# lbcb-sci/herro

Measured on NVIDIA H100. Metric: corrected_bases_per_sec, higher is better.
Workload: dtype u8 pileup/consensus + f32 forward

## Files before the change

### herro_b200/csrc/gemm_tc.cu

```cuda
#include <cstdio>
#include <cuda.h>
#include <cuda_bf16.h>

#include "common.cuh"
#include "forward.h"

namespace hb {

namespace {

constexpr int BM = 128, BN = 128, BK = 64, STAGES = 3;
constexpr int STAGE_BYTES = (2 * BM + 2 * BN) * 128;
constexpr int C_THREADS = 256, G_THREADS = 288, G_PROD_WARP = 8;

__device__ __forceinline__ uint32_t smem_u32(const void* p) { return (uint32_t)__cvta_generic_to_shared(p); }

__device__ __forceinline__ void mbar_init(uint64_t* bar, uint32_t count) {
    asm volatile("mbarrier.init.shared::cta.b64 [%0], %1;" ::"r"(smem_u32(bar)), "r"(count));
}
__device__ __forceinline__ void mbar_arrive(uint64_t* bar) {
    asm volatile("{\n\t.reg .b64 st;\n\tmbarrier.arrive.shared::cta.b64 st, [%0];\n\t}" ::"r"(smem_u32(bar)) : "memory");
}
__device__ __forceinline__ void mbar_wait(uint64_t* bar, uint32_t parity) {
    asm volatile(
        "{\n\t"
        ".reg .pred p;\n\t"
        "WAIT_LOOP:\n\t"
        "mbarrier.try_wait.parity.shared::cta.b64 p, [%0], %1;\n\t"
        "@p bra WAIT_DONE;\n\t"
        "bra WAIT_LOOP;\n\t"
        "WAIT_DONE:\n\t"
        "}" ::"r"(smem_u32(bar)), "r"(parity)
        : "memory");
}
__device__ __forceinline__ void mbar_arrive_expect_tx(uint64_t* bar, uint32_t bytes) {
    asm volatile("mbarrier.arrive.expect_tx.shared::cta.b64 _, [%0], %1;" ::"r"(smem_u32(bar)), "r"(bytes) : "memory");
}
__device__ __forceinline__ void tma_load_2d(uint32_t dst, const CUtensorMap* tm, uint64_t* bar, int c_inner, int c_row) {
    asm volatile("cp.async.bulk.tensor.2d.shared::cluster.global.mbarrier::complete_tx::bytes [%0], [%1, {%3, %4}], [%2];" ::"r"(dst),
                 "l"((uint64_t)tm), "r"(smem_u32(bar)), "r"(c_inner), "r"(c_row)
                 : "memory");
}
__device__ __forceinline__ void bar_sync(int id, int n) { asm volatile("bar.sync %0, %1;" ::"r"(id), "r"(n) : "memory"); }
__device__ __forceinline__ void fence_async_smem() { asm volatile("fence.proxy.async.shared::cta;" ::: "memory"); }

__device__ __forceinline__ uint64_t make_desc(uint32_t saddr) {
    uint64_t d = 0;
    d |= (uint64_t)((saddr & 0x3ffffu) >> 4);
    d |= (uint64_t)1 << 16;
    d |= (uint64_t)(1024u >> 4) << 32;
    d |= (uint64_t)1 << 62;
    return d;
}

__device__ __forceinline__ void wg_fence() { asm volatile("wgmma.fence.sync.aligned;" ::: "memory"); }
__device__ __forceinline__ void wg_commit() { asm volatile("wgmma.commit_group.sync.aligned;" ::: "memory"); }
template <int N>
__device__ __forceinline__ void wg_wait() { asm volatile("wgmma.wait_group.sync.aligned %0;" ::"n"(N) : "memory"); }
template <int R>
__device__ __forceinline__ void acc_fence(float (&a)[R]) {
#pragma unroll
    for (int i = 0; i < R; i++) asm volatile("" : "+f"(a[i])::"memory");
}

__device__ __forceinline__ void wgmma_n128(float (&d)[64], uint64_t adesc, uint64_t bdesc, uint32_t accumulate) {
    asm volatile(
        "{\n\t.reg .pred p;\n\tsetp.ne.b32 p, %66, 0;\n\t"
        "wgmma.mma_async.sync.aligned.m64n128k16.f32.bf16.bf16 "
        "{%0, %1, %2, %3, %4, %5, %6, %7, %8, %9, %10, %11, %12, %13, %14, %15, %16, %17, %18, %19, %20, %21, %22, %23, %24, %25, %26, %27, %28, %29, %30, %31, %32, %33, %34, %35, %36, %37, %38, %39, %40, %41, %42, %43, %44, %45, %46, %47, %48, %49, %50, %51, %52, %53, %54, %55, %56, %57, %58, %59, %60, %61, %62, %63}, "
        "%64, %65, p, 1, 1, 0, 0;\n\t}"
        : "+f"(d[0]), "+f"(d[1]), "+f"(d[2]), "+f"(d[3]), "+f"(d[4]), "+f"(d[5]), "+f"(d[6]), "+f"(d[7]), "+f"(d[8]), "+f"(d[9]), "+f"(d[10]), "+f"(d[11]), "+f"(d[12]), "+f"(d[13]), "+f"(d[14]), "+f"(d[15]), "+f"(d[16]), "+f"(d[17]), "+f"(d[18]), "+f"(d[19]), "+f"(d[20]), "+f"(d[21]), "+f"(d[22]), "+f"(d[23]), "+f"(d[24]), "+f"(d[25]), "+f"(d[26]), "+f"(d[27]), "+f"(d[28]), "+f"(d[29]), "+f"(d[30]), "+f"(d[31]), "+f"(d[32]), "+f"(d[33]), "+f"(d[34]), "+f"(d[35]), "+f"(d[36]), "+f"(d[37]), "+f"(d[38]), "+f"(d[39]), "+f"(d[40]), "+f"(d[41]), "+f"(d[42]), "+f"(d[43]), "+f"(d[44]), "+f"(d[45]), "+f"(d[46]), "+f"(d[47]), "+f"(d[48]), "+f"(d[49]), "+f"(d[50]), "+f"(d[51]), "+f"(d[52]), "+f"(d[53]), "+f"(d[54]), "+f"(d[55]), "+f"(d[56]), "+f"(d[57]), "+f"(d[58]), "+f"(d[59]), "+f"(d[60]), "+f"(d[61]), "+f"(d[62]), "+f"(d[63])
        : "l"(adesc), "l"(bdesc), "r"(accumulate)
        : "memory");
}
__device__ __forceinline__ void wgmma_n128_ra(float (&d)[64], uint32_t a0, uint32_t a1, uint32_t a2, uint32_t a3, uint64_t bdesc) {
    asm volatile(
        "wgmma.mma_async.sync.aligned.m64n128k16.f32.bf16.bf16 "
        "{%0, %1, %2, %3, %4, %5, %6, %7, %8, %9, %10, %11, %12, %13, %14, %15, %16, %17, %18, %19, %20, %21, %22, %23, %24, %25, %26, %27, %28, %29, %30, %31, %32, %33, %34, %35, %36, %37, %38, %39, %40, %41, %42, %43, %44, %45, %46, %47, %48, %49, %50, %51, %52, %53, %54, %55, %56, %57, %58, %59, %60, %61, %62, %63}, "
        "{%64, %65, %66, %67}, %68, 1, 1, 1, 0;"
        : "+f"(d[0]), "+f"(d[1]), "+f"(d[2]), "+f"(d[3]), "+f"(d[4]), "+f"(d[5]), "+f"(d[6]), "+f"(d[7]), "+f"(d[8]), "+f"(d[9]), "+f"(d[10]), "+f"(d[11]), "+f"(d[12]), "+f"(d[13]), "+f"(d[14]), "+f"(d[15]), "+f"(d[16]), "+f"(d[17]), "+f"(d[18]), "+f"(d[19]), "+f"(d[20]), "+f"(d[21]), "+f"(d[22]), "+f"(d[23]), "+f"(d[24]), "+f"(d[25]), "+f"(d[26]), "+f"(d[27]), "+f"(d[28]), "+f"(d[29]), "+f"(d[30]), "+f"(d[31]), "+f"(d[32]), "+f"(d[33]), "+f"(d[34]), "+f"(d[35]), "+f"(d[36]), "+f"(d[37]), "+f"(d[38]), "+f"(d[39]), "+f"(d[40]), "+f"(d[41]), "+f"(d[42]), "+f"(d[43]), "+f"(d[44]), "+f"(d[45]), "+f"(d[46]), "+f"(d[47]), "+f"(d[48]), "+f"(d[49]), "+f"(d[50]), "+f"(d[51]), "+f"(d[52]), "+f"(d[53]), "+f"(d[54]), "+f"(d[55]), "+f"(d[56]), "+f"(d[57]), "+f"(d[58]), "+f"(d[59]), "+f"(d[60]), "+f"(d[61]), "+f"(d[62]), "+f"(d[63])
        : "r"(a0), "r"(a1), "r"(a2), "r"(a3), "l"(bdesc)
        : "memory");
}
__device__ __forceinline__ void wgmma_n96(float (&d)[48], uint64_t adesc, uint64_t bdesc, uint32_t accumulate) {
    asm volatile(
        "{\n\t.reg .pred p;\n\tsetp.ne.b32 p, %50, 0;\n\t"
        "wgmma.mma_async.sync.aligned.m64n96k16.f32.bf16.bf16 "
        "{%0, %1, %2, %3, %4, %5, %6, %7, %8, %9, %10, %11, %12, %13, %14, %15, %16, %17, %18, %19, %20, %21, %22, %23, %24, %25, %26, %27, %28, %29, %30, %31, %32, %33, %34, %35, %36, %37, %38, %39, %40, %41, %42, %43, %44, %45, %46, %47}, "
        "%48, %49, p, 1, 1, 0, 0;\n\t}"
        : "+f"(d[0]), "+f"(d[1]), "+f"(d[2]), "+f"(d[3]), "+f"(d[4]), "+f"(d[5]), "+f"(d[6]), "+f"(d[7]), "+f"(d[8]), "+f"(d[9]), "+f"(d[10]), "+f"(d[11]), "+f"(d[12]), "+f"(d[13]), "+f"(d[14]), "+f"(d[15]), "+f"(d[16]), "+f"(d[17]), "+f"(d[18]), "+f"(d[19]), "+f"(d[20]), "+f"(d[21]), "+f"(d[22]), "+f"(d[23]), "+f"(d[24]), "+f"(d[25]), "+f"(d[26]), "+f"(d[27]), "+f"(d[28]), "+f"(d[29]), "+f"(d[30]), "+f"(d[31]), "+f"(d[32]), "+f"(d[33]), "+f"(d[34]), "+f"(d[35]), "+f"(d[36]), "+f"(d[37]), "+f"(d[38]), "+f"(d[39]), "+f"(d[40]), "+f"(d[41]), "+f"(d[42]), "+f"(d[43]), "+f"(d[44]), "+f"(d[45]), "+f"(d[46]), "+f"(d[47])
        : "l"(adesc), "l"(bdesc), "r"(accumulate)
        : "memory");
}

__device__ __forceinline__ void mma_kblock(float (&acc)[64], uint32_t a_hi, uint32_t a_lo, uint32_t b_hi, uint32_t b_lo, bool zero) {
    const uint64_t dAh = make_desc(a_hi), dAl = make_desc(a_lo), dBh = make_desc(b_hi), dBl = make_desc(b_lo);
// ... 319 lines not shown
        if (FUSE_O) {
            issue(accO, 0, true);
            issue(accO, 1, true);
            ffn_retire<1>(empty_bar, it_stage);
            acc_fence(accO);
#pragma unroll
            for (int j = 0; j < 16; j++) {
                const int c = 8 * j + fc;
                const float2 x0 = xr[2 * j], x1 = xr[2 * j + 1];
                accO[4 * j] = accO[4 * j] + s_bo[c] + x0.x; accO[4 * j + 1] = accO[4 * j + 1] + s_bo[c + 1] + x0.y;
                accO[4 * j + 2] = accO[4 * j + 2] + s_bo[c] + x1.x; accO[4 * j + 3] = accO[4 * j + 3] + s_bo[c + 1] + x1.y;
            }
            float ln[4];
            frag_ln_stats(accO, ln[0], ln[1], ln[2], ln[3]);
            bar_sync(1 + wg, 128);
            frag_store_tile(accO, sA1, fr, fc, s_ln2g, s_ln2b, ln);
#pragma unroll
            for (int j = 0; j < 16; j++) {
                const int c = 8 * j + fc;
                accO[4 * j] += s_b2[c]; accO[4 * j + 1] += s_b2[c + 1]; accO[4 * j + 2] += s_b2[c]; accO[4 * j + 3] += s_b2[c + 1];
            }
            fence_async_smem();
            bar_sync(1 + wg, 128);
        }
        issue(accF, 0, true);
        issue(accF, 1, true);
        ffn_retire<1>(empty_bar, it_stage);
        acc_fence(accF);
        e1(0);
        for (int c = 0; c < 3; c++) {
            issue_f2();
            issue(accF, 0, true);
            issue(accF, 1, true);
            ffn_retire<3>(empty_bar, it_stage);
            acc_fence(accF);
            reg_fence(ahi);
            reg_fence(alo);
            if (c == 2) mbar_arrive(&a1_empty);
            e1(c + 1);
        }
        issue_f2();
        ffn_retire<1>(empty_bar, it_stage);
        acc_fence(accO);
        reg_fence(ahi);
        reg_fence(alo);
        if (g.store_x) frag_store_f32(accO, g.X, BN, row0, 0, fc);
        frag_layernorm(accO, s_lng, s_lnb, fc);
        frag_store_split(accO, g.out_hi, g.out_lo, BN, row0, 0, fc);
    }
}

constexpr int QA_HROWS = 96;
constexpr int QA_RING_BYTES = 2 * QA_HROWS * 128;
constexpr int QA_STAGES = 3;
constexpr int QA_POS_BYTES = 6 * 2048;

__device__ __forceinline__ void ldsm_x4(uint32_t addr, uint32_t (&r)[4]) {
    asm volatile("ldmatrix.sync.aligned.m8n8.x4.shared.b16 {%0, %1, %2, %3}, [%4];" : "=r"(r[0]), "=r"(r[1]), "=r"(r[2]), "=r"(r[3]) : "r"(addr));
}
__device__ __forceinline__ void ldsm_x4_trans(uint32_t addr, uint32_t (&r)[4]) {
    asm volatile("ldmatrix.sync.aligned.m8n8.x4.trans.shared.b16 {%0, %1, %2, %3}, [%4];" : "=r"(r[0]), "=r"(r[1]), "=r"(r[2]), "=r"(r[3]) : "r"(addr));
}
__device__ __forceinline__ void mma16816(float (&c)[4], const uint32_t (&a)[4], uint32_t b0, uint32_t b1) {
    asm volatile("mma.sync.aligned.m16n8k16.row.col.f32.bf16.bf16.f32 {%0, %1, %2, %3}, {%4, %5, %6, %7}, {%8, %9}, {%0, %1, %2, %3};"
                 : "+f"(c[0]), "+f"(c[1]), "+f"(c[2]), "+f"(c[3])
                 : "r"(a[0]), "r"(a[1]), "r"(a[2]), "r"(a[3]), "r"(b0), "r"(b1));
}
__device__ __forceinline__ uint32_t qa_off(int row, int chunk) { return (uint32_t)(row * 64 + ((chunk ^ ((row >> 1) & 3)) << 4)); }

__global__ void __launch_bounds__(G_THREADS, 1) k_qkv_attn_ws(QkvAttnArgs g, const __grid_constant__ CUtensorMap tmHhi,
                                                             const __grid_constant__ CUtensorMap tmHlo, const __grid_constant__ CUtensorMap tmWhi,
                                                             const __grid_constant__ CUtensorMap tmWlo) {
    extern __shared__ uint8_t smem_dyn[];
    uint8_t* smem = smem_dyn + ((1024u - (smem_u32(smem_dyn) & 1023u)) & 1023u);
    uint8_t* sA = smem;
    uint8_t* ring = sA + FFN_A_BYTES;
    uint8_t* sP = ring + QA_STAGES * QA_RING_BYTES;
    __shared__ uint64_t full_bar[QA_STAGES], empty_bar[QA_STAGES], a_full, a_empty;
    __shared__ __align__(16) float s_bias[4 * QA_HROWS];

    const int tid = threadIdx.x, warp = tid >> 5, lane = tid & 31;
    if (tid == 0) {
        for (int s = 0; s < QA_STAGES; s++) { mbar_init(&full_bar[s], 1); mbar_init(&empty_bar[s], C_THREADS); }
        mbar_init(&a_full, 1); mbar_init(&a_empty, C_THREADS);
        asm volatile("fence.mbarrier_init.release.cluster;" ::: "memory");
    }
    for (int i = tid; i < 4 * QA_HROWS; i += G_THREADS) s_bias[i] = g.bias[i];
    __syncthreads();

    if (warp == G_PROD_WARP) {
        if (lane == 0) {
            uint32_t it_stage = 0, n_done = 0;
            for (uint32_t tile = blockIdx.x; tile < g.m_tiles; tile += gridDim.x, n_done++) {
                const int m0 = (int)(tile * BM);
                mbar_wait(&a_empty, (n_done & 1) ^ 1);
                mbar_arrive_expect_tx(&a_full, FFN_A_BYTES);
                for (int kb = 0; kb < 2; kb++) {
                    tma_load_2d(smem_u32(sA) + kb * (2 * BM * 128), &tmHhi, &a_full, kb * BK, m0);
                    tma_load_2d(smem_u32(sA) + kb * (2 * BM * 128) + BM * 128, &tmHlo, &a_full, kb * BK, m0);
                }
                for (int h = 0; h < 4; h++)
                    for (int kb = 0; kb < 2; kb++, it_stage++) {
                        const uint32_t s = it_stage % QA_STAGES, ph = (it_stage / QA_STAGES) & 1;
                        mbar_wait(&empty_bar[s], ph ^ 1);
                        const uint32_t sb = smem_u32(ring + (size_t)s * QA_RING_BYTES);
                        mbar_arrive_expect_tx(&full_bar[s], QA_RING_BYTES);
                        tma_load_2d(sb, &tmWhi, &full_bar[s], kb * BK, h * QA_HROWS);
                        tma_load_2d(sb + QA_HROWS * 128, &tmWlo, &full_bar[s], kb * BK, h * QA_HROWS);
                    }
            }
        }
        return;
    }
    const int wg = warp >> 2;
    const int pos = wg * 2 + ((warp & 3) >> 1);
    const int mt = warp & 1;
    const int gq = lane >> 2, tq = lane & 3;
    uint8_t* pb = sP + (size_t)pos * QA_POS_BYTES;
    uint8_t *aQh = pb, *aQl = pb + 2048, *aKh = pb + 4096, *aKl = pb + 6144, *aVh = pb + 8192, *aVl = pb + 10240;
    const uint32_t uQh = smem_u32(aQh), uQl = smem_u32(aQl), uKh = smem_u32(aKh), uKl = smem_u32(aKl), uVh = smem_u32(aVh),
                   uVl = smem_u32(aVl);
    const float scale_l2 = rsqrtf(32.f) * 1.4426950408889634f;
    const uint32_t ab = smem_u32(sA) + wg * 64 * 128;
    uint32_t it_stage = 0, n_done = 0;
    for (uint32_t tile = blockIdx.x; tile < g.m_tiles; tile += gridDim.x, n_done++) {
        mbar_wait(&a_full, n_done & 1);
        for (int h = 0; h < 4; h++) {
            float acc[48];
            for (int kb = 0; kb < 2; kb++, it_stage++) {
                const uint32_t s = it_stage % QA_STAGES, ph = (it_stage / QA_STAGES) & 1;
                mbar_wait(&full_bar[s], ph);
                const uint32_t sb = smem_u32(ring + (size_t)s * QA_RING_BYTES);
                const uint32_t a = ab + kb * (2 * BM * 128);
                const uint64_t dAh = make_desc(a), dAl = make_desc(a + BM * 128), dBh = make_desc(sb), dBl = make_desc(sb + QA_HROWS * 128);
                wg_fence();
#pragma unroll
                for (int k = 0; k < BK / 16; k++) {
                    const uint64_t adv = (uint64_t)(k * 2);
                    wgmma_n96(acc, dAh + adv, dBh + adv, (kb | k) ? 1u : 0u);
                    wgmma_n96(acc, dAl + adv, dBh + adv, 1u);
                    wgmma_n96(acc, dAh + adv, dBl + adv, 1u);
                }
                wg_commit();
            }
            wg_wait<0>();
            acc_fence(acc);
            mbar_arrive(&empty_bar[(it_stage - 2) % QA_STAGES]);
            mbar_arrive(&empty_bar[(it_stage - 1) % QA_STAGES]);
            if (h == 3) mbar_arrive(&a_empty);
            bar_sync(3 + pos, 64);
            const float* bb = s_bias + h * QA_HROWS;
#pragma unroll
            for (int j = 0; j < 12; j++) {
                const int c = 8 * j + 2 * tq;
                const float sc = j < 4 ? scale_l2 : 1.f;
                uint8_t* hi_arr = j < 4 ? aQh : (j < 8 ? aKh : aVh);
                const int cc = c & 31;
#pragma unroll
                for (int hf = 0; hf < 2; hf++) {
                    const int row = mt * 16 + hf * 8 + gq;
                    uint32_t hw, lw;
                    split2((acc[4 * j + 2 * hf] + bb[c]) * sc, (acc[4 * j + 2 * hf + 1] + bb[c + 1]) * sc, hw, lw);
                    const uint32_t off = qa_off(row, cc >> 3) + (cc & 7) * 2;
                    *(uint32_t*)(hi_arr + off) = hw;
                    *(uint32_t*)(hi_arr + 2048 + off) = lw;
                }
            }
            bar_sync(3 + pos, 64);
            float sacc[4][4];
#pragma unroll
            for (int nt = 0; nt < 4; nt++)
#pragma unroll
                for (int e = 0; e < 4; e++) sacc[nt][e] = 0.f;
            {
                uint32_t qh[2][4], ql[2][4];
#pragma unroll
                for (int ks = 0; ks < 2; ks++) {
                    const uint32_t off = qa_off(mt * 16 + (lane & 7) + ((lane >> 3) & 1) * 8, ks * 2 + (lane >> 4));
                    ldsm_x4(uQh + off, qh[ks]);
                    ldsm_x4(uQl + off, ql[ks]);
                }
#pragma unroll
                for (int ntp = 0; ntp < 2; ntp++)
#pragma unroll
                    for (int ks = 0; ks < 2; ks++) {
                        uint32_t kh[4], kl[4];
                        const uint32_t off = qa_off(ntp * 16 + (lane & 7) + (lane >> 4) * 8, ks * 2 + ((lane >> 3) & 1));
                        ldsm_x4(uKh + off, kh);
                        ldsm_x4(uKl + off, kl);
#pragma unroll
                        for (int j = 0; j < 2; j++) {
                            mma16816(sacc[ntp * 2 + j], qh[ks], kh[2 * j], kh[2 * j + 1]);
                            mma16816(sacc[ntp * 2 + j], ql[ks], kh[2 * j], kh[2 * j + 1]);
                            mma16816(sacc[ntp * 2 + j], qh[ks], kl[2 * j], kl[2 * j + 1]);
                        }
                    }
            }
            float inv[2];
#pragma unroll
            for (int hf = 0; hf < 2; hf++) {
                if (tq == 3) sacc[3][2 * hf + 1] = -INFINITY;
                float m = -INFINITY;
#pragma unroll
                for (int nt = 0; nt < 4; nt++) m = fmaxf(m, fmaxf(sacc[nt][2 * hf], sacc[nt][2 * hf + 1]));
                m = fmaxf(m, __shfl_xor_sync(HB_FULL, m, 1));
                m = fmaxf(m, __shfl_xor_sync(HB_FULL, m, 2));
                float l = 0.f;
#pragma unroll
                for (int nt = 0; nt < 4; nt++) {
                    const float p0 = exp2f(sacc[nt][2 * hf] - m), p1 = exp2f(sacc[nt][2 * hf + 1] - m);
                    sacc[nt][2 * hf] = p0; sacc[nt][2 * hf + 1] = p1;
                    l += p0 + p1;
                }
                l += __shfl_xor_sync(HB_FULL, l, 1);
                l += __shfl_xor_sync(HB_FULL, l, 2);
                const int row = mt * 16 + hf * 8 + gq;
                inv[hf] = (row < R_COLS) ? 1.f / l : 0.f;
            }
            float oacc[4][4];
#pragma unroll
            for (int dt = 0; dt < 4; dt++)
#pragma unroll
                for (int e = 0; e < 4; e++) oacc[dt][e] = 0.f;
#pragma unroll
            for (int ks = 0; ks < 2; ks++) {
                uint32_t ph[4], pl[4];
                split2(sacc[2 * ks][0], sacc[2 * ks][1], ph[0], pl[0]);
                split2(sacc[2 * ks][2], sacc[2 * ks][3], ph[1], pl[1]);
                split2(sacc[2 * ks + 1][0], sacc[2 * ks + 1][1], ph[2], pl[2]);
                split2(sacc[2 * ks + 1][2], sacc[2 * ks + 1][3], ph[3], pl[3]);
#pragma unroll
                for (int dp = 0; dp < 2; dp++) {
                    uint32_t vh[4], vl[4];
                    const uint32_t off = qa_off(ks * 16 + (lane & 7) + ((lane >> 3) & 1) * 8, dp * 2 + (lane >> 4));
                    ldsm_x4_trans(uVh + off, vh);
                    ldsm_x4_trans(uVl + off, vl);
#pragma unroll
                    for (int j = 0; j < 2; j++) {
                        mma16816(oacc[dp * 2 + j], ph, vh[2 * j], vh[2 * j + 1]);
                        mma16816(oacc[dp * 2 + j], pl, vh[2 * j], vh[2 * j + 1]);
                        mma16816(oacc[dp * 2 + j], ph, vl[2 * j], vl[2 * j + 1]);
                    }
                }
            }
            uint32_t* sth = (uint32_t*)aQh;
            uint32_t* stl = (uint32_t*)aQl;
            __syncwarp();
#pragma unroll
            for (int hf = 0; hf < 2; hf++) {
                const int row = mt * 16 + hf * 8 + gq;
#pragma unroll
                for (int dt = 0; dt < 4; dt++) {
                    uint32_t hi, lo;
                    split2(oacc[dt][2 * hf] * inv[hf], oacc[dt][2 * hf + 1] * inv[hf], hi, lo);
                    const int w = row * 16 + ((dt ^ ((row >> 1) & 3)) << 2) + tq;
                    sth[w] = hi;
                    stl[w] = lo;
                }
            }
            __syncwarp();
            const size_t rb = ((size_t)tile * BM + pos * 32) * BN + h * 32;
#pragma unroll
            for (int jj = 0; jj < 2; jj++) {
                const int rr = mt * 16 + jj * 8 + (lane >> 2), cq = lane & 3;
                const int w = rr * 16 + ((cq ^ ((rr >> 1) & 3)) << 2);
                *(uint4*)(g.out_hi + rb + (size_t)rr * BN + cq * 8) = *(const uint4*)(sth + w);
                *(uint4*)(g.out_lo + rb + (size_t)rr * BN + cq * 8) = *(const uint4*)(stl + w);
            }
            __syncwarp();
        }
    }
}

constexpr int STEM_STAGE_BYTES = (BM + 2 * BN) * 128;
constexpr int STEM_MAXK = 64;
constexpr int STEM_RP_LD = 132;
constexpr int S_PROD = 128, S_GATHER = 64, S_THREADS = 448, S_GATHER_WARP = 12;

__global__ void __launch_bounds__(S_THREADS, 1) k_stem_tc(BatchView b, StemArgs g, const __grid_constant__ CUtensorMap tmWhi,
                                                         const __grid_constant__ CUtensorMap tmWlo) {
    extern __shared__ uint8_t smem_dyn[];
    uint8_t* smem = smem_dyn + ((1024u - (smem_u32(smem_dyn) & 1023u)) & 1023u);
    uint8_t* tokbuf = smem + STAGES * STEM_STAGE_BYTES;
    uint8_t* qbuf = tokbuf + 2 * 4 * STEM_MAXK * 32;
    float* s_rp = (float*)(qbuf + 2 * 4 * STEM_MAXK * 32);
    __shared__ uint64_t full_bar[STAGES], empty_bar[STAGES], buf_full[2], buf_empty[2];
    __shared__ __align__(16) float s_bias[BN], s_lng[BN], s_lnb[BN];

    const int tid = threadIdx.x, warp = tid >> 5, lane = tid & 31;
    if (tid < BN) {
        s_bias[tid] = g.bias[tid];
        s_lng[tid] = g.out_hi ? g.ln_g[tid] : 1.f;
        s_lnb[tid] = g.out_hi ? g.ln_b[tid] : 0.f;
    }
    for (int i = tid; i < 32 * BN; i += S_THREADS) {
        const int r = i >> 7, c = i & 127;
        s_rp[r * STEM_RP_LD + c] = r < R_COLS ? g.read_pos[i] : 0.f;
    }
    if (tid == 0) {
        for (int s = 0; s < STAGES; s++) { mbar_init(&full_bar[s], S_PROD + 1); mbar_init(&empty_bar[s], C_THREADS); }
        for (int a = 0; a < 2; a++) { mbar_init(&buf_full[a], S_GATHER); mbar_init(&buf_empty[a], S_PROD); }
        asm volatile("fence.mbarrier_init.release.cluster;" ::: "memory");
    }
    __syncthreads();
    const uint32_t n_items = (g.npos + 3) / 4;
    const uint32_t kbs = g.k_blocks;
    const int K = g.taps;

    if (warp >= 8 && warp < S_GATHER_WARP) {
        const int p = tid - C_THREADS;
        const int pos = p >> 5, rd = p & 31;
        uint32_t it_stage = 0, n_done = 0;
        for (uint32_t item = blockIdx.x; item < n_items; item += gridDim.x, n_done++) {
            const uint8_t* tb = tokbuf + (n_done & 1) * 4 * STEM_MAXK * 32;
            const uint8_t* qb = qbuf + (n_done & 1) * 4 * STEM_MAXK * 32;
            mbar_wait(&buf_full[n_done & 1], (n_done >> 1) & 1);
            const uint8_t* trow = tb + pos * STEM_MAXK * 32 + rd;
            const uint8_t* qrow = qb + pos * STEM_MAXK * 32 + rd;
            for (uint32_t kb = 0; kb < kbs; kb++, it_stage++) {
                const uint32_t s = it_stage % STAGES, ph = (it_stage / STAGES) & 1;
                mbar_wait(&empty_bar[s], ph ^ 1);
                uint8_t* sA = smem + (size_t)s * STEM_STAGE_BYTES;
                if (p == 0) {
                    mbar_arrive_expect_tx(&full_bar[s], 2 * BN * 128);
// ... 106 lines not shown
        acc_fence(acc);
        mbar_arrive(&empty_bar[prev]);
        const size_t row0 = (size_t)item * BM + fr;
#pragma unroll
        for (int j = 0; j < 16; j++) {
            const int c = 8 * j + fc;
            const float* rp0 = s_rp + rd0 * STEM_RP_LD + c;
            const float* rp1 = s_rp + rd1 * STEM_RP_LD + c;
            acc[4 * j] = fmaxf(acc[4 * j] + s_bias[c], 0.f) + rp0[0];
            acc[4 * j + 1] = fmaxf(acc[4 * j + 1] + s_bias[c + 1], 0.f) + rp0[1];
            acc[4 * j + 2] = fmaxf(acc[4 * j + 2] + s_bias[c], 0.f) + rp1[0];
            acc[4 * j + 3] = fmaxf(acc[4 * j + 3] + s_bias[c + 1], 0.f) + rp1[1];
            if (rd0 >= R_COLS) { acc[4 * j] = 0.f; acc[4 * j + 1] = 0.f; }
            if (rd1 >= R_COLS) { acc[4 * j + 2] = 0.f; acc[4 * j + 3] = 0.f; }
        }
        frag_store_f32(acc, g.X, BN, row0, 0, fc);
        if (g.out_hi) {
            frag_layernorm(acc, s_lng, s_lnb, fc);
            frag_store_split(acc, g.out_hi, g.out_lo, BN, row0, 0, fc);
        }
    }
}

__global__ void k_split_bf16(const float* __restrict__ w, __nv_bfloat16* __restrict__ hi, __nv_bfloat16* __restrict__ lo, size_t n) {
    const size_t i = (size_t)blockIdx.x * blockDim.x + threadIdx.x;
    if (i < n) {
        const __nv_bfloat16 h = __float2bfloat16_rn(w[i]);
        hi[i] = h;
        lo[i] = __float2bfloat16_rn(w[i] - __bfloat162float(h));
    }
}

cudaError_t split_weights(const float* w, size_t n, void** hi, void** lo) {
    cudaError_t e = cudaMalloc(hi, n * 2);
    if (e != cudaSuccess) return e;
    e = cudaMalloc(lo, n * 2);
    if (e != cudaSuccess) return e;
    k_split_bf16<<<(unsigned)((n + 255) / 256), 256>>>(w, (__nv_bfloat16*)*hi, (__nv_bfloat16*)*lo, n);
    return cudaGetLastError();
}

typedef CUresult (*EncodeTiledFn)(CUtensorMap*, CUtensorMapDataType, cuuint32_t, void*, const cuuint64_t*, const cuuint64_t*,
                                  const cuuint32_t*, const cuuint32_t*, CUtensorMapInterleave, CUtensorMapSwizzle,
                                  CUtensorMapL2promotion, CUtensorMapFloatOOBfill);
static EncodeTiledFn encode_fn() {
    static EncodeTiledFn fn = nullptr;
    if (!fn) {
        void* p = nullptr;
        cudaDriverEntryPointQueryResult q;
        if (cudaGetDriverEntryPoint("cuTensorMapEncodeTiled", &p, cudaEnableDefault, &q) == cudaSuccess) fn = (EncodeTiledFn)p;
    }
    return fn;
}
static bool make_tmap(CUtensorMap* tm, const void* base, uint64_t rows, uint64_t cols, uint64_t ld, uint32_t box_rows = BM) {
    EncodeTiledFn fn = encode_fn();
    if (!fn) return false;
    const cuuint64_t gdim[2] = {cols, rows};
    const cuuint64_t gstr[1] = {ld * 2};
    const cuuint32_t box[2] = {BK, box_rows};
    const cuuint32_t estr[2] = {1, 1};
    return fn(tm, CU_TENSOR_MAP_DATA_TYPE_BFLOAT16, 2, const_cast<void*>(base), gdim, gstr, box, estr, CU_TENSOR_MAP_INTERLEAVE_NONE,
              CU_TENSOR_MAP_SWIZZLE_128B, CU_TENSOR_MAP_L2_PROMOTION_L2_128B, CU_TENSOR_MAP_FLOAT_OOB_FILL_NONE) == CUDA_SUCCESS;
}

cudaError_t gemm_tc(const GemmArgs& a, int num_sms, cudaStream_t st) {
    static bool configured = false;
    const size_t smem = (size_t)STAGES * STAGE_BYTES + 1024;
    if (!configured) {
        cudaError_t e = cudaFuncSetAttribute(k_gemm_ws, cudaFuncAttributeMaxDynamicSharedMemorySize, (int)smem);
        if (e != cudaSuccess) return e;
        configured = true;
    }
    const uint32_t items = a.m_tiles * a.n_chunks;
    if (items == 0) return cudaSuccess;
    CUtensorMap tAh, tAl, tWh, tWl;
    const uint64_t M = (uint64_t)a.m_tiles * BM, N = (uint64_t)a.n_chunks * BN;
    if (!make_tmap(&tAh, a.Ahi, M, a.K, a.lda) || !make_tmap(&tAl, a.Alo, M, a.K, a.lda) || !make_tmap(&tWh, a.Whi, N, a.K, a.K) ||
        !make_tmap(&tWl, a.Wlo, N, a.K, a.K))
        return cudaErrorInvalidValue;
    const unsigned grid = (unsigned)std::min<uint32_t>(items, (uint32_t)num_sms);
    k_gemm_ws<<<grid, G_THREADS, smem, st>>>(a, tAh, tAl, tWh, tWl);
    return cudaGetLastError();
}

cudaError_t ffn_tc(const FfnArgs& a, int num_sms, cudaStream_t st) {
    static bool configured = false;
    const size_t smem = (size_t)FFN_A_BYTES + (size_t)FFN_STAGES * FFN_RING_BYTES + 1024;
    if (!configured) {
        cudaError_t e = cudaFuncSetAttribute(k_ffn_ws<false>, cudaFuncAttributeMaxDynamicSharedMemorySize, (int)smem);
        if (e != cudaSuccess) return e;
        e = cudaFuncSetAttribute(k_ffn_ws<true>, cudaFuncAttributeMaxDynamicSharedMemorySize, (int)smem);
        if (e != cudaSuccess) return e;
        configured = true;
    }
    if (a.m_tiles == 0) return cudaSuccess;
    CUtensorMap tHh, tHl, t1h, t1l, t2h, t2l, toh, tol;
    const uint64_t T = (uint64_t)a.m_tiles * BM;
    if (!make_tmap(&tHh, a.Hhi, T, BN, BN) || !make_tmap(&tHl, a.Hlo, T, BN, BN) || !make_tmap(&t1h, a.W1hi, a.F, BN, BN) ||
        !make_tmap(&t1l, a.W1lo, a.F, BN, BN) || !make_tmap(&t2h, a.W2hi, BN, a.F, a.F) || !make_tmap(&t2l, a.W2lo, BN, a.F, a.F))
        return cudaErrorInvalidValue;
    const unsigned grid = (unsigned)std::min<uint32_t>(a.m_tiles, (uint32_t)num_sms);
    if (a.Wohi) {
        if (!make_tmap(&toh, a.Wohi, BN, BN, BN) || !make_tmap(&tol, a.Wolo, BN, BN, BN)) return cudaErrorInvalidValue;
        k_ffn_ws<true><<<grid, FFN_THREADS, smem, st>>>(a, tHh, tHl, t1h, t1l, t2h, t2l, toh, tol);
    } else {
        k_ffn_ws<false><<<grid, FFN_THREADS, smem, st>>>(a, tHh, tHl, t1h, t1l, t2h, t2l, t1h, t1l);
    }
    return cudaGetLastError();
}

cudaError_t stem_tc(const BatchView& b, const StemArgs& a, int num_sms, cudaStream_t st) {
    static bool configured = false;
    const size_t smem = (size_t)STAGES * STEM_STAGE_BYTES + 2 * 2 * 4 * STEM_MAXK * 32 + (size_t)32 * STEM_RP_LD * 4 + 1024;
    if (!configured) {
        cudaError_t e = cudaFuncSetAttribute(k_stem_tc, cudaFuncAttributeMaxDynamicSharedMemorySize, (int)smem);
        if (e != cudaSuccess) return e;
        configured = true;
    }
    const uint32_t items = (a.npos + 3) / 4;
    if (items == 0) return cudaSuccess;
    CUtensorMap tWh, tWl;
    if (!make_tmap(&tWh, a.Whi, BN, a.Kp, a.Kp) || !make_tmap(&tWl, a.Wlo, BN, a.Kp, a.Kp)) return cudaErrorInvalidValue;
    k_stem_tc<<<(unsigned)std::min<uint32_t>(items, (uint32_t)num_sms), S_THREADS, smem, st>>>(b, a, tWh, tWl);
    return cudaGetLastError();
}

cudaError_t qkv_attn_tc(const QkvAttnArgs& a, int num_sms, cudaStream_t st) {
    static bool configured = false;
    const size_t smem = (size_t)FFN_A_BYTES + (size_t)QA_STAGES * QA_RING_BYTES + (size_t)4 * QA_POS_BYTES + 1024;
    if (!configured) {
        cudaError_t e = cudaFuncSetAttribute(k_qkv_attn_ws, cudaFuncAttributeMaxDynamicSharedMemorySize, (int)smem);
        if (e != cudaSuccess) return e;
        configured = true;
    }
    if (a.m_tiles == 0) return cudaSuccess;
    CUtensorMap tHh, tHl, tWh, tWl;
    const uint64_t T = (uint64_t)a.m_tiles * BM;
    if (!make_tmap(&tHh, a.Hhi, T, BN, BN) || !make_tmap(&tHl, a.Hlo, T, BN, BN) || !make_tmap(&tWh, a.Whi, 4 * QA_HROWS, BN, BN, QA_HROWS) ||
        !make_tmap(&tWl, a.Wlo, 4 * QA_HROWS, BN, BN, QA_HROWS))
        return cudaErrorInvalidValue;
    k_qkv_attn_ws<<<(unsigned)std::min<uint32_t>(a.m_tiles, (uint32_t)num_sms), G_THREADS, smem, st>>>(a, tHh, tHl, tWh, tWl);
    return cudaGetLastError();
}

}
```

Before: 551.1 million.

## Pipeline fused QKV-attention kernel with per-warpgroup H loads, ping-pong WGMMA, TMA stores

Restructures the fused QKV+attention kernel. The H tile is split into per-warpgroup halves with separate full/empty barriers, so each warpgroup can refill its half independently. Named barriers make the two warpgroups alternate their WGMMA phases so one's GEMM overlaps the other's attention math. Q fragments now stay in registers instead of going through shared memory and ldmatrix. Output goes out via asynchronous TMA bulk stores, and the weight ring deepens from 3 to 4 stages. It adds synchronisation complexity, with risks of deadlock or ordering bugs and more shared memory use.

```diff
diff --git a/herro_b200/csrc/gemm_tc.cu b/herro_b200/csrc/gemm_tc.cu
--- a/herro_b200/csrc/gemm_tc.cu
+++ b/herro_b200/csrc/gemm_tc.cu
@@ -41,7 +41,16 @@
                  "l"((uint64_t)tm), "r"(smem_u32(bar)), "r"(c_inner), "r"(c_row)
                  : "memory");
 }
+__device__ __forceinline__ void tma_store_2d(const CUtensorMap* tm, uint32_t src, int c_inner, int c_row) {
+    asm volatile("cp.async.bulk.tensor.2d.global.shared::cta.bulk_group [%0, {%2, %3}], [%1];" ::"l"((uint64_t)tm), "r"(src), "r"(c_inner),
+                 "r"(c_row)
+                 : "memory");
+}
+__device__ __forceinline__ void bulk_commit() { asm volatile("cp.async.bulk.commit_group;" ::: "memory"); }
+__device__ __forceinline__ void bulk_wait_read() { asm volatile("cp.async.bulk.wait_group.read 0;" ::: "memory"); }
+__device__ __forceinline__ void bulk_wait() { asm volatile("cp.async.bulk.wait_group 0;" ::: "memory"); }
 __device__ __forceinline__ void bar_sync(int id, int n) { asm volatile("bar.sync %0, %1;" ::"r"(id), "r"(n) : "memory"); }
+__device__ __forceinline__ void bar_arrive(int id, int n) { asm volatile("bar.arrive %0, %1;" ::"r"(id), "r"(n) : "memory"); }
 __device__ __forceinline__ void fence_async_smem() { asm volatile("fence.proxy.async.shared::cta;" ::: "memory"); }
 
 __device__ __forceinline__ uint64_t make_desc(uint32_t saddr) {
@@ -467,8 +476,9 @@
 
 constexpr int QA_HROWS = 96;
 constexpr int QA_RING_BYTES = 2 * QA_HROWS * 128;
-constexpr int QA_STAGES = 3;
+constexpr int QA_STAGES = 4;
 constexpr int QA_POS_BYTES = 6 * 2048;
+constexpr int QA_BAR_WG0 = 7, QA_BAR_WG1 = 8;
 
 __device__ __forceinline__ void ldsm_x4(uint32_t addr, uint32_t (&r)[4]) {
     asm volatile("ldmatrix.sync.aligned.m8n8.x4.shared.b16 {%0, %1, %2, %3}, [%4];" : "=r"(r[0]), "=r"(r[1]), "=r"(r[2]), "=r"(r[3]) : "r"(addr));
@@ -485,36 +495,32 @@
 
 __global__ void __launch_bounds__(G_THREADS, 1) k_qkv_attn_ws(QkvAttnArgs g, const __grid_constant__ CUtensorMap tmHhi,
                                                              const __grid_constant__ CUtensorMap tmHlo, const __grid_constant__ CUtensorMap tmWhi,
-                                                             const __grid_constant__ CUtensorMap tmWlo) {
+                                                             const __grid_constant__ CUtensorMap tmWlo, const __grid_constant__ CUtensorMap tmOhi,
+                                                             const __grid_constant__ CUtensorMap tmOlo) {
     extern __shared__ uint8_t smem_dyn[];
     uint8_t* smem = smem_dyn + ((1024u - (smem_u32(smem_dyn) & 1023u)) & 1023u);
     uint8_t* sA = smem;
     uint8_t* ring = sA + FFN_A_BYTES;
     uint8_t* sP = ring + QA_STAGES * QA_RING_BYTES;
-    __shared__ uint64_t full_bar[QA_STAGES], empty_bar[QA_STAGES], a_full, a_empty;
+    __shared__ uint64_t full_bar[QA_STAGES], empty_bar[QA_STAGES], h_full[2], h_empty[2];
     __shared__ __align__(16) float s_bias[4 * QA_HROWS];
 
     const int tid = threadIdx.x, warp = tid >> 5, lane = tid & 31;
     if (tid == 0) {
         for (int s = 0; s < QA_STAGES; s++) { mbar_init(&full_bar[s], 1); mbar_init(&empty_bar[s], C_THREADS); }
-        mbar_init(&a_full, 1); mbar_init(&a_empty, C_THREADS);
+        for (int w = 0; w < 2; w++) { mbar_init(&h_full[w], 1); mbar_init(&h_empty[w], C_THREADS / 2); }
         asm volatile("fence.mbarrier_init.release.cluster;" ::: "memory");
     }
     for (int i = tid; i < 4 * QA_HROWS; i += G_THREADS) s_bias[i] = g.bias[i];
     __syncthreads();
+    const uint32_t n_tiles = (g.m_tiles - blockIdx.x + gridDim.x - 1) / gridDim.x;
 
     if (warp == G_PROD_WARP) {
         if (lane == 0) {
-            uint32_t it_stage = 0, n_done = 0;
-            for (uint32_t tile = blockIdx.x; tile < g.m_tiles; tile += gridDim.x, n_done++) {
+            uint32_t it_stage = 0;
+            for (uint32_t n = 0, tile = blockIdx.x; n < n_tiles; n++, tile += gridDim.x) {
                 const int m0 = (int)(tile * BM);
-                mbar_wait(&a_empty, (n_done & 1) ^ 1);
-                mbar_arrive_expect_tx(&a_full, FFN_A_BYTES);
-                for (int kb = 0; kb < 2; kb++) {
-                    tma_load_2d(smem_u32(sA) + kb * (2 * BM * 128), &tmHhi, &a_full, kb * BK, m0);
-                    tma_load_2d(smem_u32(sA) + kb * (2 * BM * 128) + BM * 128, &tmHlo, &a_full, kb * BK, m0);
-                }
-                for (int h = 0; h < 4; h++)
+                for (int h = 0; h < 4; h++) {
                     for (int kb = 0; kb < 2; kb++, it_stage++) {
                         const uint32_t s = it_stage % QA_STAGES, ph = (it_stage / QA_STAGES) & 1;
                         mbar_wait(&empty_bar[s], ph ^ 1);
@@ -523,6 +529,17 @@
                         tma_load_2d(sb, &tmWhi, &full_bar[s], kb * BK, h * QA_HROWS);
                         tma_load_2d(sb + QA_HROWS * 128, &tmWlo, &full_bar[s], kb * BK, h * QA_HROWS);
                     }
+                    if (h == 0)
+                        for (int w = 0; w < 2; w++) {
+                            mbar_wait(&h_empty[w], (n & 1) ^ 1);
+                            mbar_arrive_expect_tx(&h_full[w], FFN_A_BYTES / 2);
+                            for (int kb = 0; kb < 2; kb++) {
+                                const uint32_t d = smem_u32(sA) + kb * (2 * BM * 128) + w * 64 * 128;
+                                tma_load_2d(d, &tmHhi, &h_full[w], kb * BK, m0 + 64 * w);
+                                tma_load_2d(d + BM * 128, &tmHlo, &h_full[w], kb * BK, m0 + 64 * w);
+                            }
+                        }
+                }
             }
         }
         return;
@@ -532,16 +549,18 @@
     const int mt = warp & 1;
     const int gq = lane >> 2, tq = lane & 3;
     uint8_t* pb = sP + (size_t)pos * QA_POS_BYTES;
-    uint8_t *aQh = pb, *aQl = pb + 2048, *aKh = pb + 4096, *aKl = pb + 6144, *aVh = pb + 8192, *aVl = pb + 10240;
-    const uint32_t uQh = smem_u32(aQh), uQl = smem_u32(aQl), uKh = smem_u32(aKh), uKl = smem_u32(aKl), uVh = smem_u32(aVh),
-                   uVl = smem_u32(aVl);
+    uint8_t *aOh = pb, *aOl = pb + 2048, *aKh = pb + 4096, *aVh = pb + 8192;
+    const uint32_t uKh = smem_u32(aKh), uKl = uKh + 2048, uVh = smem_u32(aVh), uVl = uVh + 2048;
     const float scale_l2 = rsqrtf(32.f) * 1.4426950408889634f;
     const uint32_t ab = smem_u32(sA) + wg * 64 * 128;
-    uint32_t it_stage = 0, n_done = 0;
-    for (uint32_t tile = blockIdx.x; tile < g.m_tiles; tile += gridDim.x, n_done++) {
-        mbar_wait(&a_full, n_done & 1);
-        for (int h = 0; h < 4; h++) {
+    const uint32_t n_heads = 4 * n_tiles;
+    uint32_t it_stage = 0, i_head = 0;
+    for (uint32_t n = 0, tile = blockIdx.x; n < n_tiles; n++, tile += gridDim.x) {
+        mbar_wait(&h_full[wg], n & 1);
+        for (int h = 0; h < 4; h++, i_head++) {
             float acc[48];
+            if (wg == 1) bar_sync(QA_BAR_WG1, C_THREADS);
+            else if (i_head > 0) bar_sync(QA_BAR_WG0, C_THREADS);
             for (int kb = 0; kb < 2; kb++, it_stage++) {
                 const uint32_t s = it_stage % QA_STAGES, ph = (it_stage / QA_STAGES) & 1;
                 mbar_wait(&full_bar[s], ph);
@@ -558,27 +577,35 @@
                 }
                 wg_commit();
             }
+            if (wg == 0) bar_arrive(QA_BAR_WG1, C_THREADS);
+            else if (i_head + 1 < n_heads) bar_arrive(QA_BAR_WG0, C_THREADS);
             wg_wait<0>();
             acc_fence(acc);
             mbar_arrive(&empty_bar[(it_stage - 2) % QA_STAGES]);
             mbar_arrive(&empty_bar[(it_stage - 1) % QA_STAGES]);
-            if (h == 3) mbar_arrive(&a_empty);
+            if (h == 3) mbar_arrive(&h_empty[wg]);
+            uint32_t qh[2][4], ql[2][4];
             bar_sync(3 + pos, 64);
             const float* bb = s_bias + h * QA_HROWS;
 #pragma unroll
             for (int j = 0; j < 12; j++) {
                 const int c = 8 * j + 2 * tq;
                 const float sc = j < 4 ? scale_l2 : 1.f;
-                uint8_t* hi_arr = j < 4 ? aQh : (j < 8 ? aKh : aVh);
+                uint8_t* hi_arr = j < 8 ? aKh : aVh;
                 const int cc = c & 31;
 #pragma unroll
                 for (int hf = 0; hf < 2; hf++) {
                     const int row = mt * 16 + hf * 8 + gq;
                     uint32_t hw, lw;
                     split2((acc[4 * j + 2 * hf] + bb[c]) * sc, (acc[4 * j + 2 * hf + 1] + bb[c + 1]) * sc, hw, lw);
-                    const uint32_t off = qa_off(row, cc >> 3) + (cc & 7) * 2;
-                    *(uint32_t*)(hi_arr + off) = hw;
-                    *(uint32_t*)(hi_arr + 2048 + off) = lw;
+                    if (j < 4) {
+                        qh[j >> 1][(j & 1) * 2 + hf] = hw;
+                        ql[j >> 1][(j & 1) * 2 + hf] = lw;
+                    } else {
+                        const uint32_t off = qa_off(row, cc >> 3) + (cc & 7) * 2;
+                        *(uint32_t*)(hi_arr + off) = hw;
+                        *(uint32_t*)(hi_arr + 2048 + off) = lw;
+                    }
                 }
             }
             bar_sync(3 + pos, 64);
@@ -588,13 +615,6 @@
 #pragma unroll
                 for (int e = 0; e < 4; e++) sacc[nt][e] = 0.f;
             {
-                uint32_t qh[2][4], ql[2][4];
-#pragma unroll
-                for (int ks = 0; ks < 2; ks++) {
-                    const uint32_t off = qa_off(mt * 16 + (lane & 7) + ((lane >> 3) & 1) * 8, ks * 2 + (lane >> 4));
-                    ldsm_x4(uQh + off, qh[ks]);
-                    ldsm_x4(uQl + off, ql[ks]);
-                }
 #pragma unroll
                 for (int ntp = 0; ntp < 2; ntp++)
 #pragma unroll
@@ -658,8 +678,9 @@
                     }
                 }
             }
-            uint32_t* sth = (uint32_t*)aQh;
-            uint32_t* stl = (uint32_t*)aQl;
+            uint32_t* sth = (uint32_t*)aOh;
+            uint32_t* stl = (uint32_t*)aOl;
+            if (lane == 0) bulk_wait_read();
             __syncwarp();
 #pragma unroll
             for (int hf = 0; hf < 2; hf++) {
@@ -673,18 +694,17 @@
                     stl[w] = lo;
                 }
             }
+            fence_async_smem();
             __syncwarp();
-            const size_t rb = ((size_t)tile * BM + pos * 32) * BN + h * 32;
-#pragma unroll
-            for (int jj = 0; jj < 2; jj++) {
-                const int rr = mt * 16 + jj * 8 + (lane >> 2), cq = lane & 3;
-                const int w = rr * 16 + ((cq ^ ((rr >> 1) & 3)) << 2);
-                *(uint4*)(g.out_hi + rb + (size_t)rr * BN + cq * 8) = *(const uint4*)(sth + w);
-                *(uint4*)(g.out_lo + rb + (size_t)rr * BN + cq * 8) = *(const uint4*)(stl + w);
-            }
-            __syncwarp();
-        }
-    }
+            if (lane == 0) {
+                const int r0 = (int)(tile * BM) + pos * 32 + mt * 16;
+                tma_store_2d(&tmOhi, smem_u32(sth) + mt * 16 * 64, h * 32, r0);
+                tma_store_2d(&tmOlo, smem_u32(stl) + mt * 16 * 64, h * 32, r0);
+                bulk_commit();
+            }
+        }
+    }
+    if (lane == 0) bulk_wait();
 }
 
 constexpr int STEM_STAGE_BYTES = (BM + 2 * BN) * 128;
@@ -897,15 +917,16 @@
     }
     return fn;
 }
-static bool make_tmap(CUtensorMap* tm, const void* base, uint64_t rows, uint64_t cols, uint64_t ld, uint32_t box_rows = BM) {
+static bool make_tmap(CUtensorMap* tm, const void* base, uint64_t rows, uint64_t cols, uint64_t ld, uint32_t box_rows = BM,
+                      uint32_t box_cols = BK, CUtensorMapSwizzle swizzle = CU_TENSOR_MAP_SWIZZLE_128B) {
     EncodeTiledFn fn = encode_fn();
     if (!fn) return false;
     const cuuint64_t gdim[2] = {cols, rows};
     const cuuint64_t gstr[1] = {ld * 2};
-    const cuuint32_t box[2] = {BK, box_rows};
+    const cuuint32_t box[2] = {box_cols, box_rows};
     const cuuint32_t estr[2] = {1, 1};
     return fn(tm, CU_TENSOR_MAP_DATA_TYPE_BFLOAT16, 2, const_cast<void*>(base), gdim, gstr, box, estr, CU_TENSOR_MAP_INTERLEAVE_NONE,
-              CU_TENSOR_MAP_SWIZZLE_128B, CU_TENSOR_MAP_L2_PROMOTION_L2_128B, CU_TENSOR_MAP_FLOAT_OOB_FILL_NONE) == CUDA_SUCCESS;
+              swizzle, CU_TENSOR_MAP_L2_PROMOTION_L2_128B, CU_TENSOR_MAP_FLOAT_OOB_FILL_NONE) == CUDA_SUCCESS;
 }
 
 cudaError_t gemm_tc(const GemmArgs& a, int num_sms, cudaStream_t st) {
@@ -979,12 +1000,14 @@
         configured = true;
     }
     if (a.m_tiles == 0) return cudaSuccess;
-    CUtensorMap tHh, tHl, tWh, tWl;
+    CUtensorMap tHh, tHl, tWh, tWl, tOh, tOl;
     const uint64_t T = (uint64_t)a.m_tiles * BM;
-    if (!make_tmap(&tHh, a.Hhi, T, BN, BN) || !make_tmap(&tHl, a.Hlo, T, BN, BN) || !make_tmap(&tWh, a.Whi, 4 * QA_HROWS, BN, BN, QA_HROWS) ||
-        !make_tmap(&tWl, a.Wlo, 4 * QA_HROWS, BN, BN, QA_HROWS))
+    if (!make_tmap(&tHh, a.Hhi, T, BN, BN, BM / 2) || !make_tmap(&tHl, a.Hlo, T, BN, BN, BM / 2) ||
+        !make_tmap(&tWh, a.Whi, 4 * QA_HROWS, BN, BN, QA_HROWS) ||
+        !make_tmap(&tWl, a.Wlo, 4 * QA_HROWS, BN, BN, QA_HROWS) ||
+        !make_tmap(&tOh, a.out_hi, T, BN, BN, 16, 32, CU_TENSOR_MAP_SWIZZLE_64B) || !make_tmap(&tOl, a.out_lo, T, BN, BN, 16, 32, CU_TENSOR_MAP_SWIZZLE_64B))
         return cudaErrorInvalidValue;
-    k_qkv_attn_ws<<<(unsigned)std::min<uint32_t>(a.m_tiles, (uint32_t)num_sms), G_THREADS, smem, st>>>(a, tHh, tHl, tWh, tWl);
+    k_qkv_attn_ws<<<(unsigned)std::min<uint32_t>(a.m_tiles, (uint32_t)num_sms), G_THREADS, smem, st>>>(a, tHh, tHl, tWh, tWl, tOh, tOl);
     return cudaGetLastError();
 }
 
```

Measured after the change: 554.2 million (median of 6 runs). No clear change (+0.6%).

## Split QKV projection and attention into separate warp roles with double-buffered staging

Applied to the files above, without the earlier changes.

The fused QKV+attention kernel now uses dedicated warps. Two warpgroups run the wgmma QKV projection and write Q/K/V into one of two shared-memory staging sets. A new set of 8 attention warps consumes those sets under per-position mbarrier handoff, so projection of the next head can overlap attention on the current one. The weight ring drops from 3 to 2 stages to make room for the doubled staging buffers, the producer prefetches the next tile's activations into L2, and the first stage's empty barrier is released earlier. The cost is more threads, more register pressure and a shallower weight pipeline.

```diff
diff --git a/herro_b200/csrc/gemm_tc.cu b/herro_b200/csrc/gemm_tc.cu
--- a/herro_b200/csrc/gemm_tc.cu
+++ b/herro_b200/csrc/gemm_tc.cu
@@ -467,8 +467,9 @@
 
 constexpr int QA_HROWS = 96;
 constexpr int QA_RING_BYTES = 2 * QA_HROWS * 128;
-constexpr int QA_STAGES = 3;
+constexpr int QA_STAGES = 2;
 constexpr int QA_POS_BYTES = 6 * 2048;
+constexpr int QA_THREADS = 544, QA_ATT_WARP = 8, QA_PROD_WARP = 16;
 
 __device__ __forceinline__ void ldsm_x4(uint32_t addr, uint32_t (&r)[4]) {
     asm volatile("ldmatrix.sync.aligned.m8n8.x4.shared.b16 {%0, %1, %2, %3}, [%4];" : "=r"(r[0]), "=r"(r[1]), "=r"(r[2]), "=r"(r[3]) : "r"(addr));
@@ -481,29 +482,33 @@
                  : "+f"(c[0]), "+f"(c[1]), "+f"(c[2]), "+f"(c[3])
                  : "r"(a[0]), "r"(a[1]), "r"(a[2]), "r"(a[3]), "r"(b0), "r"(b1));
 }
+__device__ __forceinline__ void tma_prefetch_2d(const CUtensorMap* tm, int c_inner, int c_row) {
+    asm volatile("cp.async.bulk.prefetch.tensor.2d.L2.global.tile [%0, {%1, %2}];" ::"l"((uint64_t)tm), "r"(c_inner), "r"(c_row) : "memory");
+}
 __device__ __forceinline__ uint32_t qa_off(int row, int chunk) { return (uint32_t)(row * 64 + ((chunk ^ ((row >> 1) & 3)) << 4)); }
 
-__global__ void __launch_bounds__(G_THREADS, 1) k_qkv_attn_ws(QkvAttnArgs g, const __grid_constant__ CUtensorMap tmHhi,
-                                                             const __grid_constant__ CUtensorMap tmHlo, const __grid_constant__ CUtensorMap tmWhi,
-                                                             const __grid_constant__ CUtensorMap tmWlo) {
+__global__ void __launch_bounds__(QA_THREADS, 1) k_qkv_attn_ws(QkvAttnArgs g, const __grid_constant__ CUtensorMap tmHhi,
+                                                               const __grid_constant__ CUtensorMap tmHlo, const __grid_constant__ CUtensorMap tmWhi,
+                                                               const __grid_constant__ CUtensorMap tmWlo) {
     extern __shared__ uint8_t smem_dyn[];
     uint8_t* smem = smem_dyn + ((1024u - (smem_u32(smem_dyn) & 1023u)) & 1023u);
     uint8_t* sA = smem;
     uint8_t* ring = sA + FFN_A_BYTES;
     uint8_t* sP = ring + QA_STAGES * QA_RING_BYTES;
-    __shared__ uint64_t full_bar[QA_STAGES], empty_bar[QA_STAGES], a_full, a_empty;
+    __shared__ uint64_t full_bar[QA_STAGES], empty_bar[QA_STAGES], a_full, a_empty, set_full[2][4], set_empty[2][4];
     __shared__ __align__(16) float s_bias[4 * QA_HROWS];
 
     const int tid = threadIdx.x, warp = tid >> 5, lane = tid & 31;
     if (tid == 0) {
         for (int s = 0; s < QA_STAGES; s++) { mbar_init(&full_bar[s], 1); mbar_init(&empty_bar[s], C_THREADS); }
         mbar_init(&a_full, 1); mbar_init(&a_empty, C_THREADS);
+        for (int i = 0; i < 8; i++) { mbar_init(&set_full[i >> 2][i & 3], 64); mbar_init(&set_empty[i >> 2][i & 3], 64); }
         asm volatile("fence.mbarrier_init.release.cluster;" ::: "memory");
     }
-    for (int i = tid; i < 4 * QA_HROWS; i += G_THREADS) s_bias[i] = g.bias[i];
+    for (int i = tid; i < 4 * QA_HROWS; i += QA_THREADS) s_bias[i] = g.bias[i];
     __syncthreads();
 
-    if (warp == G_PROD_WARP) {
+    if (warp == QA_PROD_WARP) {
         if (lane == 0) {
             uint32_t it_stage = 0, n_done = 0;
             for (uint32_t tile = blockIdx.x; tile < g.m_tiles; tile += gridDim.x, n_done++) {
@@ -514,6 +519,11 @@
                     tma_load_2d(smem_u32(sA) + kb * (2 * BM * 128), &tmHhi, &a_full, kb * BK, m0);
                     tma_load_2d(smem_u32(sA) + kb * (2 * BM * 128) + BM * 128, &tmHlo, &a_full, kb * BK, m0);
                 }
+                if (tile + gridDim.x < g.m_tiles)
+                    for (int kb = 0; kb < 2; kb++) {
+                        tma_prefetch_2d(&tmHhi, kb * BK, m0 + (int)(gridDim.x * BM));
+                        tma_prefetch_2d(&tmHlo, kb * BK, m0 + (int)(gridDim.x * BM));
+                    }
                 for (int h = 0; h < 4; h++)
                     for (int kb = 0; kb < 2; kb++, it_stage++) {
                         const uint32_t s = it_stage % QA_STAGES, ph = (it_stage / QA_STAGES) & 1;
@@ -527,61 +537,76 @@
         }
         return;
     }
-    const int wg = warp >> 2;
-    const int pos = wg * 2 + ((warp & 3) >> 1);
+    const int gq = lane >> 2, tq = lane & 3;
+    if (warp < QA_ATT_WARP) {
+        const int wg = warp >> 2;
+        const int pos = wg * 2 + ((warp & 3) >> 1);
+        const int mt = warp & 1;
+        const float scale_l2 = rsqrtf(32.f) * 1.4426950408889634f;
+        const uint32_t ab = smem_u32(sA) + wg * 64 * 128;
+        uint32_t it_stage = 0, n_done = 0, hc = 0;
+        for (uint32_t tile = blockIdx.x; tile < g.m_tiles; tile += gridDim.x, n_done++) {
+            mbar_wait(&a_full, n_done & 1);
+            for (int h = 0; h < 4; h++, hc++) {
+                float acc[48];
+                for (int kb = 0; kb < 2; kb++, it_stage++) {
+                    const uint32_t s = it_stage % QA_STAGES, ph = (it_stage / QA_STAGES) & 1;
+                    mbar_wait(&full_bar[s], ph);
+                    const uint32_t sb = smem_u32(ring + (size_t)s * QA_RING_BYTES);
+                    const uint32_t a = ab + kb * (2 * BM * 128);
+                    const uint64_t dAh = make_desc(a), dAl = make_desc(a + BM * 128), dBh = make_desc(sb), dBl = make_desc(sb + QA_HROWS * 128);
+                    wg_fence();
+#pragma unroll
+                    for (int k = 0; k < BK / 16; k++) {
+                        const uint64_t adv = (uint64_t)(k * 2);
+                        wgmma_n96(acc, dAh + adv, dBh + adv, (kb | k) ? 1u : 0u);
+                        wgmma_n96(acc, dAl + adv, dBh + adv, 1u);
+                        wgmma_n96(acc, dAh + adv, dBl + adv, 1u);
+                    }
+                    wg_commit();
+                }
+                wg_wait<1>();
+                mbar_arrive(&empty_bar[(it_stage - 2) % QA_STAGES]);
+                wg_wait<0>();
+                acc_fence(acc);
+                mbar_arrive(&empty_bar[(it_stage - 1) % QA_STAGES]);
+                if (h == 3) mbar_arrive(&a_empty);
+                const uint32_t set = hc & 1;
+                uint8_t* pb = sP + (size_t)(set * 4 + pos) * QA_POS_BYTES;
+                uint8_t *aQh = pb, *aKh = pb + 4096, *aVh = pb + 8192;
+                mbar_wait(&set_empty[set][pos], ((hc >> 1) & 1) ^ 1);
+                const float* bb = s_bias + h * QA_HROWS;
+#pragma unroll
+                for (int j = 0; j < 12; j++) {
+                    const int c = 8 * j + 2 * tq;
+                    const float sc = j < 4 ? scale_l2 : 1.f;
+                    uint8_t* hi_arr = j < 4 ? aQh : (j < 8 ? aKh : aVh);
+                    const int cc = c & 31;
+#pragma unroll
+                    for (int hf = 0; hf < 2; hf++) {
+                        const int row = mt * 16 + hf * 8 + gq;
+                        uint32_t hw, lw;
+                        split2((acc[4 * j + 2 * hf] + bb[c]) * sc, (acc[4 * j + 2 * hf + 1] + bb[c + 1]) * sc, hw, lw);
+                        const uint32_t off = qa_off(row, cc >> 3) + (cc & 7) * 2;
+                        *(uint32_t*)(hi_arr + off) = hw;
+                        *(uint32_t*)(hi_arr + 2048 + off) = lw;
+                    }
+                }
+                mbar_arrive(&set_full[set][pos]);
+            }
+        }
+        return;
+    }
+    const int pos = (warp - QA_ATT_WARP) >> 1;
     const int mt = warp & 1;
-    const int gq = lane >> 2, tq = lane & 3;
-    uint8_t* pb = sP + (size_t)pos * QA_POS_BYTES;
-    uint8_t *aQh = pb, *aQl = pb + 2048, *aKh = pb + 4096, *aKl = pb + 6144, *aVh = pb + 8192, *aVl = pb + 10240;
-    const uint32_t uQh = smem_u32(aQh), uQl = smem_u32(aQl), uKh = smem_u32(aKh), uKl = smem_u32(aKl), uVh = smem_u32(aVh),
-                   uVl = smem_u32(aVl);
-    const float scale_l2 = rsqrtf(32.f) * 1.4426950408889634f;
-    const uint32_t ab = smem_u32(sA) + wg * 64 * 128;
-    uint32_t it_stage = 0, n_done = 0;
-    for (uint32_t tile = blockIdx.x; tile < g.m_tiles; tile += gridDim.x, n_done++) {
-        mbar_wait(&a_full, n_done & 1);
-        for (int h = 0; h < 4; h++) {
-            float acc[48];
-            for (int kb = 0; kb < 2; kb++, it_stage++) {
-                const uint32_t s = it_stage % QA_STAGES, ph = (it_stage / QA_STAGES) & 1;
-                mbar_wait(&full_bar[s], ph);
-                const uint32_t sb = smem_u32(ring + (size_t)s * QA_RING_BYTES);
-                const uint32_t a = ab + kb * (2 * BM * 128);
-                const uint64_t dAh = make_desc(a), dAl = make_desc(a + BM * 128), dBh = make_desc(sb), dBl = make_desc(sb + QA_HROWS * 128);
-                wg_fence();
-#pragma unroll
-                for (int k = 0; k < BK / 16; k++) {
-                    const uint64_t adv = (uint64_t)(k * 2);
-                    wgmma_n96(acc, dAh + adv, dBh + adv, (kb | k) ? 1u : 0u);
-                    wgmma_n96(acc, dAl + adv, dBh + adv, 1u);
-                    wgmma_n96(acc, dAh + adv, dBl + adv, 1u);
-                }
-                wg_commit();
-            }
-            wg_wait<0>();
-            acc_fence(acc);
-            mbar_arrive(&empty_bar[(it_stage - 2) % QA_STAGES]);
-            mbar_arrive(&empty_bar[(it_stage - 1) % QA_STAGES]);
-            if (h == 3) mbar_arrive(&a_empty);
-            bar_sync(3 + pos, 64);
-            const float* bb = s_bias + h * QA_HROWS;
-#pragma unroll
-            for (int j = 0; j < 12; j++) {
-                const int c = 8 * j + 2 * tq;
-                const float sc = j < 4 ? scale_l2 : 1.f;
-                uint8_t* hi_arr = j < 4 ? aQh : (j < 8 ? aKh : aVh);
-                const int cc = c & 31;
-#pragma unroll
-                for (int hf = 0; hf < 2; hf++) {
-                    const int row = mt * 16 + hf * 8 + gq;
-                    uint32_t hw, lw;
-                    split2((acc[4 * j + 2 * hf] + bb[c]) * sc, (acc[4 * j + 2 * hf + 1] + bb[c + 1]) * sc, hw, lw);
-                    const uint32_t off = qa_off(row, cc >> 3) + (cc & 7) * 2;
-                    *(uint32_t*)(hi_arr + off) = hw;
-                    *(uint32_t*)(hi_arr + 2048 + off) = lw;
-                }
-            }
-            bar_sync(3 + pos, 64);
+    uint32_t hc = 0;
+    for (uint32_t tile = blockIdx.x; tile < g.m_tiles; tile += gridDim.x) {
+        for (int h = 0; h < 4; h++, hc++) {
+            const uint32_t set = hc & 1;
+            uint8_t* pb = sP + (size_t)(set * 4 + pos) * QA_POS_BYTES;
+            uint8_t *aQh = pb, *aQl = pb + 2048;
+            const uint32_t uQh = smem_u32(aQh), uQl = uQh + 2048, uKh = uQh + 4096, uKl = uQh + 6144, uVh = uQh + 8192, uVl = uQh + 10240;
+            mbar_wait(&set_full[set][pos], (hc >> 1) & 1);
             float sacc[4][4];
 #pragma unroll
             for (int nt = 0; nt < 4; nt++)
@@ -682,7 +707,7 @@
                 *(uint4*)(g.out_hi + rb + (size_t)rr * BN + cq * 8) = *(const uint4*)(sth + w);
                 *(uint4*)(g.out_lo + rb + (size_t)rr * BN + cq * 8) = *(const uint4*)(stl + w);
             }
-            __syncwarp();
+            mbar_arrive(&set_empty[set][pos]);
         }
     }
 }
@@ -972,7 +997,7 @@
 
 cudaError_t qkv_attn_tc(const QkvAttnArgs& a, int num_sms, cudaStream_t st) {
     static bool configured = false;
-    const size_t smem = (size_t)FFN_A_BYTES + (size_t)QA_STAGES * QA_RING_BYTES + (size_t)4 * QA_POS_BYTES + 1024;
+    const size_t smem = (size_t)FFN_A_BYTES + (size_t)QA_STAGES * QA_RING_BYTES + (size_t)2 * 4 * QA_POS_BYTES + 1024;
     if (!configured) {
         cudaError_t e = cudaFuncSetAttribute(k_qkv_attn_ws, cudaFuncAttributeMaxDynamicSharedMemorySize, (int)smem);
         if (e != cudaSuccess) return e;
@@ -984,7 +1009,7 @@
     if (!make_tmap(&tHh, a.Hhi, T, BN, BN) || !make_tmap(&tHl, a.Hlo, T, BN, BN) || !make_tmap(&tWh, a.Whi, 4 * QA_HROWS, BN, BN, QA_HROWS) ||
         !make_tmap(&tWl, a.Wlo, 4 * QA_HROWS, BN, BN, QA_HROWS))
         return cudaErrorInvalidValue;
-    k_qkv_attn_ws<<<(unsigned)std::min<uint32_t>(a.m_tiles, (uint32_t)num_sms), G_THREADS, smem, st>>>(a, tHh, tHl, tWh, tWl);
+    k_qkv_attn_ws<<<(unsigned)std::min<uint32_t>(a.m_tiles, (uint32_t)num_sms), QA_THREADS, smem, st>>>(a, tHh, tHl, tWh, tWl);
     return cudaGetLastError();
 }
 
```

Result: faster. 553.8 million before, 562.1 million after, median of 6 (+1.5%).
